# Human-Augment-Analytics/vectordb-retrieval

Measured on AMD Instinct MI355X. Metric: QPS @ recall@10 (SIFT1M-shaped, 10k-query batch, k=10), higher is better.
Workload: dtype i8 MFMA scan (i32 accumulate) + exact integer / f64 refine

## Files before the change

vectordb-retrieval_amd/csrc/scan_i8x16.hpp:

```cpp
#pragma once
#include "scan_i8.hpp"

namespace vdb {

__host__ __device__ inline int x16_row_in_span(int t, int rb, int m) { return (m >> 2) * 128 + t * 8 + rb * 4 + (m & 3); }

__device__ __forceinline__ int swap16(int v) { return __builtin_amdgcn_ds_swizzle(v, 0x401F); }

template <int KS2, int ST, int RING>
constexpr int scan_i8x16_lds_bytes() { return RING * (ST * 2 * KS2 * 64 * 16 + ST * 32 * 4); }

template <int KS2, int ST, int CB, int NWAVES = 8, int RING = 2, int AUX = 0>
__device__ __forceinline__ void scan_i8x16_body(const ScanI8Args &a, unsigned char *smem) {
    constexpr int NV = 2 * KS2;
    constexpr int NT = NWAVES * 64;
    constexpr int kStageVec = ST * NV * 64;
    constexpr int kBiasLoads = (ST * 32 + NT - 1) / NT;
    constexpr int TPS = kTilesPerSpan;
    constexpr int SPS = TPS / ST;
    constexpr int HC = CB / 2;
    constexpr int UNR = (ST * CB <= 16) ? ST : 1;
    static_assert(TPS % ST == 0 && ST >= 2 && CB % 2 == 0 && NWAVES <= 8, "bad geometry");
    static_assert(RING >= 2 && RING <= 8 && (RING == 2 || ST % 2 == 0), "bad ring");
    constexpr bool kDeep = RING > 2;
    static_assert(scan_i8x16_lds_bytes<KS2, ST, RING>() == RING * (kStageVec * 16 + ST * 32 * 4), "LDS size");
    const int mode = a.info->i8_mode;
    if (!mode) return;
    auto lds_a = [&](int buf) { return reinterpret_cast<int4v *>(smem + buf * (kStageVec * 16)); };
    auto lds_b = [&](int buf) { return reinterpret_cast<int *>(smem + RING * kStageVec * 16 + buf * (ST * 32 * 4)); };

    const int tid = threadIdx.x, lane = tid & 63;
    const int wave = __builtin_amdgcn_readfirstlane(tid >> 6);
    const int g = lane >> 4, h = g >> 1;
    const bool odd = (g & 1) != 0;
    const bool late = (NWAVES >= 2) && (wave >= NWAVES / 2);
    const int b = blockIdx.x;
    const int x = b & 7, jb = b >> 3;
    const int ci = jb / a.nqtiles, qt = jb - ci * a.nqtiles;
    const int chunk = x + 8 * ci;
    if (chunk >= a.nchunks) return;
    const int64_t q0 = (int64_t)qt * (NWAVES * 16 * CB) + wave * (16 * CB);
    const int64_t span0 = chunk_span0(chunk, a.spans_per_chunk, a.chunk_rem);
    int64_t span1 = chunk_span0(chunk + 1, a.spans_per_chunk, a.chunk_rem);
    if (span1 > a.nspans) span1 = a.nspans;
    const int64_t out_pitch = a.Qpad;
    const int64_t col0 = q0 + (odd ? 16 : 0) + (lane & 15);
    const int32_t *bias = a.bias8 + ((mode & 3) == 1 ? 0 : a.Npad);

    int4v bq[CB][KS2];
#pragma unroll
    for (int cb = 0; cb < CB; ++cb)
#pragma unroll
        for (int ks = 0; ks < KS2; ++ks) bq[cb][ks] = a.qpanels[((size_t)(q0 / 16 + cb) * KS2 + ks) * 64 + lane];
    const int nstages = (int)(span1 - span0) * SPS;
    const int INF = (int)kI8Inf;
    int m1[CB], m2[CB], M1[HC], M2[HC], Ms[HC];
#pragma unroll
    for (int cb = 0; cb < CB; ++cb) m1[cb] = m2[cb] = INF;
#pragma unroll
    for (int j = 0; j < HC; ++j) {
        M1[j] = M2[j] = INF;
        Ms[j] = 0;
    }

    constexpr int kPieces = kStageVec / 64;
    static_assert(kPieces % NWAVES == 0, "pieces must divide over the waves");
    constexpr int kBiasPieces = (ST / 2 + NWAVES - 1) / NWAVES;
    int stage_b[kBiasLoads];
    auto stage_issue = [&](int st, int buf) {
        const int64_t span = span0 + st / SPS;
        const int sq = st % SPS;
        const int4v *src = a.panels + ((size_t)(span * TPS + sq * ST) * NV) * 64;
        int4v *dst = lds_a(buf);
#pragma unroll
        for (int i = 0; i < kPieces / NWAVES; ++i) {
            const int p = wave + i * NWAVES;
            const int4v *gp = src + p * 64 + lane;
            __builtin_amdgcn_global_load_lds(
                reinterpret_cast<const __attribute__((address_space(1))) void *>(reinterpret_cast<uintptr_t>(gp)),
                reinterpret_cast<__attribute__((address_space(3))) void *>(
                    static_cast<uint32_t>(reinterpret_cast<uintptr_t>(dst + p * 64))),
                16, 0, AUX);
        }
        if (kDeep) {
#pragma unroll
            for (int i = 0; i < kBiasPieces; ++i) {
                const int j = (wave + i * NWAVES) % (ST / 2);
                const int t = 2 * j + (lane >> 5), gg = (lane >> 3) & 3, e = lane & 7;
                const int32_t *gp = bias + span * kSpanRows + gg * 128 + (sq * ST + t) * 8 + e;
                __builtin_amdgcn_global_load_lds(
                    reinterpret_cast<const __attribute__((address_space(1))) void *>(reinterpret_cast<uintptr_t>(gp)),
                    reinterpret_cast<__attribute__((address_space(3))) void *>(
                        static_cast<uint32_t>(reinterpret_cast<uintptr_t>(lds_b(buf) + j * 64))),
                    4, 0, 0);
            }
            return;
        }
#pragma unroll
        for (int i = 0; i < kBiasLoads; ++i) {
            const int e = tid + i * NT;
            if (e < ST * 32) {
                const int t = e >> 5, gg = (e >> 3) & 3, r = e & 7;
                stage_b[i] = bias[span * kSpanRows + gg * 128 + (sq * ST + t) * 8 + r];
            }
        }
    };
    auto stage_bias_store = [&](int buf) {
        if (kDeep) return;
#pragma unroll
        for (int i = 0; i < kBiasLoads; ++i)
            if (tid + i * NT < ST * 32) lds_b(buf)[tid + i * NT] = stage_b[i];
    };
    auto ring_issue = [&](int st) { stage_issue(st < nstages ? st : nstages - 1, st % RING); };
    auto ring_wait = [&]() {
        constexpr int kKeep = (RING - 2) * (kPieces / NWAVES + kBiasPieces);
        static_assert(kKeep < 64, "vmcnt is a 6-bit counter");
        asm volatile("s_waitcnt vmcnt(%0)" ::"n"(kKeep) : "memory");
        __builtin_amdgcn_s_barrier();
        asm volatile("" ::: "memory");
    };
    auto flush_bin = [&](int64_t span) {
        const size_t o = (size_t)(span * 2 + h) * out_pitch + col0;
#pragma unroll
        for (int j = 0; j < HC; ++j) {
            const int p1 = swap16(odd ? m1[2 * j] : m1[2 * j + 1]), p2 = swap16(odd ? m2[2 * j] : m2[2 * j + 1]);
            const int a1 = odd ? m1[2 * j + 1] : m1[2 * j], a2 = odd ? m2[2 * j + 1] : m2[2 * j];
            const int b1 = imin(a1, p1), b2 = imin(imax(a1, p1), imin(a2, p2));
            __builtin_nontemporal_store(__int_as_float(b1), a.bin_m1 + o + j * 32);
            __builtin_nontemporal_store(__int_as_float(b2), a.bin_m2 + o + j * 32);
            M2[j] = imin(imed3(M1[j], M2[j], b1), b2);
            if (b1 < M1[j]) Ms[j] = (int)span;
            M1[j] = imin(M1[j], b1);
        }
#pragma unroll
        for (int cb = 0; cb < CB; ++cb) m1[cb] = m2[cb] = INF;
    };

    if (kDeep) {
#pragma unroll
        for (int s = 0; s < RING - 1; ++s) ring_issue(s);
    } else {
        stage_issue(0, 0);
    }
    stage_bias_store(0);
    if (kDeep) ring_wait();
    else __syncthreads();

    if (a.nq_valid > 0 && q0 >= a.nq_valid) {
        for (int st = 0; st < nstages; ++st) {
            if (kDeep) {
                ring_issue(st + RING - 1);
                ring_wait();
                continue;
            }
            if (st + 1 < nstages) {
                stage_issue(st + 1, (st & 1) ^ 1);
                stage_bias_store((st & 1) ^ 1);
            }
            __syncthreads();
        }
        return;
    }

    int4v fr[NV], cin[2], acc[2][CB];
    auto read_phase = [&](const int4v *A_tile, const int4v *c_tile) {
#pragma unroll
        for (int v = 0; v < NV; ++v) fr[v] = A_tile[v * 64 + lane];
        cin[0] = c_tile[0];
        cin[1] = c_tile[1];
    };
    auto mfma_phase = [&]() {
#pragma unroll
        for (int ks = 0; ks < KS2; ++ks)
#pragma unroll
            for (int rb = 0; rb < 2; ++rb)
#pragma unroll
                for (int cb = 0; cb < CB; ++cb)
                    acc[rb][cb] = __builtin_amdgcn_mfma_i32_16x16x64_i8(fr[2 * ks + rb], bq[cb][ks], ks == 0 ? cin[rb] : acc[rb][cb], 0, 0, 0);
    };
    const unsigned id_hi = odd ? 16u : 0u;
    auto select_phase = [&](int t_bin) {
        const unsigned idv = (unsigned)__builtin_amdgcn_readfirstlane(t_bin) | id_hi;
#pragma unroll
        for (int cb = 0; cb < CB; ++cb) {
            const int t1 = imin(imin(acc[0][cb][0], acc[0][cb][1]), acc[0][cb][2]);
            const int t2 = imin(imin(acc[0][cb][3], acc[1][cb][0]), acc[1][cb][1]);
            const int q = imin(imin(imin(acc[1][cb][2], acc[1][cb][3]), t1), t2);
            const int v = (int)(((unsigned)q << 6) | idv);
            m2[cb] = imed3(m1[cb], m2[cb], v);
            m1[cb] = imin(m1[cb], v);
        }
    };
    if (a.prio == 1 && late) __builtin_amdgcn_s_setprio(1);
    else if (a.prio == 2 && !late) __builtin_amdgcn_s_setprio(1);
    if (!late) {
        for (int st = 0; st < nstages; ++st) {
            const int buf = kDeep ? st % RING : st & 1;
            if (kDeep) ring_issue(st + RING - 1);
            else if (st + 1 < nstages) stage_issue(st + 1, buf ^ 1);
            const int4v *A = lds_a(buf);
            const int4v *B4 = reinterpret_cast<const int4v *>(lds_b(buf)) + g * 2;
            const int ts0 = (st % SPS) * ST;
            read_phase(A, B4);
#pragma unroll UNR
            for (int t = 0; t < ST; ++t) {
                __builtin_amdgcn_sched_barrier(0);
                mfma_phase();
                __builtin_amdgcn_sched_barrier(0);
                if (t + 1 < ST) read_phase(A + (t + 1) * NV * 64, B4 + (t + 1) * 8);
                select_phase(ts0 + t);
            }
            __builtin_amdgcn_sched_barrier(0);
            if (ts0 + ST == TPS) flush_bin(span0 + st / SPS);
            if (!kDeep && st + 1 < nstages) stage_bias_store(buf ^ 1);
            if (kDeep) ring_wait();
            else __syncthreads();
        }
    } else {
#pragma unroll
        for (int rb = 0; rb < 2; ++rb)
#pragma unroll
            for (int cb = 0; cb < CB; ++cb)
#pragma unroll
                for (int r = 0; r < 4; ++r) acc[rb][cb][r] = (int)(kI8Inf >> 6);
        for (int st = 0; st < nstages; ++st) {
            const int buf = kDeep ? st % RING : st & 1;
            if (kDeep) ring_issue(st + RING - 1);
            else if (st + 1 < nstages) stage_issue(st + 1, buf ^ 1);
            const int4v *A = lds_a(buf);
            const int4v *B4 = reinterpret_cast<const int4v *>(lds_b(buf)) + g * 2;
            const int ts0 = (st % SPS) * ST;
#pragma unroll UNR
            for (int t = 0; t < ST; ++t) {
                __builtin_amdgcn_sched_barrier(0);
                read_phase(A + t * NV * 64, B4 + t * 8);
                select_phase((ts0 + t + TPS - 1) % TPS);
                if (t == 0 && st > 0 && ts0 == 0) flush_bin(span0 + st / SPS - 1);
                __builtin_amdgcn_sched_barrier(0);
                mfma_phase();
            }
            __builtin_amdgcn_sched_barrier(0);
            if (!kDeep && st + 1 < nstages) stage_bias_store(buf ^ 1);
            if (kDeep) ring_wait();
            else __syncthreads();
        }
        select_phase(TPS - 1);
        flush_bin(span1 - 1);
    }

    const size_t so = (size_t)(chunk * 2 + h) * a.Qpad + col0;
#pragma unroll
    for (int j = 0; j < HC; ++j) {
        a.sb_m1[so + j * 32] = __int_as_float(M1[j]);
        a.sb_m2[so + j * 32] = __int_as_float(M2[j]);
        a.sb_span[so + j * 32] = Ms[j];
    }
}

template <int KS2, int ST, int CB, int NWAVES = 8, int RING = 2, int AUX = 0>
__global__ __launch_bounds__(NWAVES * 64, (NWAVES >= 4 ? 2 : 1)) void scan_i8x16_kernel(ScanI8Args a) {
    __shared__ __attribute__((aligned(16))) unsigned char smem[scan_i8x16_lds_bytes<KS2, ST, RING>()];
    scan_i8x16_body<KS2, ST, CB, NWAVES, RING, AUX>(a, smem);
}

}
```

Measured before the change: 11.40 million.

## Software-pipeline i8x16 scan tiles with double-buffered accumulators and interleaved MFMA schedule

Adds a specialized batch loop for the 8-wave, 2-ring, non-unrolled configuration. Accumulators and fragments are double-buffered so the min-reduction and top-2 folds of the previous tile, plus the LDS reads for the next tile, interleave with the MFMAs of the current tile. sched_group_barrier patterns place VALU and DS ops into MFMA gaps. This aims to hide the select/fold VALU work and LDS latency behind matrix ops, at the cost of roughly doubling accumulator and fragment register use, which may reduce occupancy or cause spills.

```diff
diff --git a/vectordb-retrieval_amd/csrc/scan_i8x16.hpp b/vectordb-retrieval_amd/csrc/scan_i8x16.hpp
--- a/vectordb-retrieval_amd/csrc/scan_i8x16.hpp
+++ b/vectordb-retrieval_amd/csrc/scan_i8x16.hpp
@@ -9,6 +9,105 @@
 
 template <int KS2, int ST, int RING>
 constexpr int scan_i8x16_lds_bytes() { return RING * (ST * 2 * KS2 * 64 * 16 + ST * 32 * 4); }
+
+template <int N_MFMA, int N_VALU, int N_DS>
+__device__ __forceinline__ void x16_gap_pattern() {
+    constexpr int R = (N_VALU + N_DS + N_MFMA - 1) / N_MFMA;
+    static_assert(N_DS <= N_MFMA && R >= 2, "one LDS read per gap");
+#pragma unroll
+    for (int i = 0; i < N_MFMA; ++i) {
+        __builtin_amdgcn_sched_group_barrier(0x8, 1, 0);
+        if (i < N_DS) {
+            __builtin_amdgcn_sched_group_barrier(0x100, 1, 0);
+            __builtin_amdgcn_sched_group_barrier(0x2, R - 1, 0);
+        } else {
+            __builtin_amdgcn_sched_group_barrier(0x2, R, 0);
+        }
+    }
+}
+
+template <int KS2, int ST, int CB, class StageIssue, class BiasStore, class FlushBin>
+__device__ __forceinline__ void scan_i8x16_batch_loop(const unsigned char *smem, const int4v (&bq)[CB][KS2], int (&m1)[CB], int (&m2)[CB],
+                                                      int nstages, int64_t span0, int lane, StageIssue &&stage_issue,
+                                                      BiasStore &&stage_bias_store, FlushBin &&flush_bin) {
+    constexpr int NV = 2 * KS2, kStageVec = ST * NV * 64, TPS = kTilesPerSpan, SPS = TPS / ST;
+    constexpr int NM = 2 * KS2 * CB, NH = NM / 2;
+    static_assert(ST % 2 == 0 && TPS % ST == 0, "tile parity must be static in the unrolled stage");
+    const int g = lane >> 4;
+    const unsigned id_hi = (g & 1) ? 16u : 0u;
+    int4v acc[2][2][CB], fr[2][NV], cin[2][2];
+    int q[CB];
+#pragma unroll
+    for (int rb = 0; rb < 2; ++rb)
+#pragma unroll
+        for (int cb = 0; cb < CB; ++cb)
+#pragma unroll
+            for (int r = 0; r < 4; ++r) acc[1][rb][cb][r] = (int)(kI8Inf >> 6);
+    auto read_tile = [&](int p, const int4v *A, const int4v *B4, int t) {
+#pragma unroll
+        for (int v = 0; v < NV; ++v) fr[p][v] = A[(t * NV + v) * 64];
+        cin[p][0] = B4[t * 8];
+        cin[p][1] = B4[t * 8 + 1];
+    };
+    auto mfma_half = [&](int p, int half) {
+#pragma unroll
+        for (int m = half * NH; m < (half + 1) * NH; ++m) {
+            const int ks = m / (2 * CB), rb = (m / CB) % 2, cb = m % CB;
+            acc[p][rb][cb] = __builtin_amdgcn_mfma_i32_16x16x64_i8(fr[p][2 * ks + rb], bq[cb][ks], ks == 0 ? cin[p][rb] : acc[p][rb][cb], 0, 0, 0);
+        }
+    };
+    auto min_trees = [&](int o) {
+#pragma unroll
+        for (int cb = 0; cb < CB; ++cb) {
+            const int t1 = imin(imin(acc[o][0][cb][0], acc[o][0][cb][1]), acc[o][0][cb][2]);
+            const int t2 = imin(imin(acc[o][0][cb][3], acc[o][1][cb][0]), acc[o][1][cb][1]);
+            q[cb] = imin(imin(imin(acc[o][1][cb][2], acc[o][1][cb][3]), t1), t2);
+        }
+    };
+    auto folds = [&](int t_bin) {
+        const unsigned idv = (unsigned)__builtin_amdgcn_readfirstlane(t_bin) | id_hi;
+#pragma unroll
+        for (int cb = 0; cb < CB; ++cb) {
+            const int v = (int)(((unsigned)q[cb] << 6) | idv);
+            m2[cb] = imed3(m1[cb], m2[cb], v);
+            m1[cb] = imin(m1[cb], v);
+        }
+    };
+    for (int st = 0; st < nstages; ++st) {
+        const int buf = st & 1;
+        if (st + 1 < nstages) stage_issue(st + 1, buf ^ 1);
+        const int4v *A = reinterpret_cast<const int4v *>(smem + buf * (kStageVec * 16)) + lane;
+        const int4v *B4 = reinterpret_cast<const int4v *>(smem + 2 * kStageVec * 16 + buf * (ST * 32 * 4)) + g * 2;
+        const int ts0 = (st % SPS) * ST;
+        read_tile(0, A, B4, 0);
+#pragma unroll
+        for (int t = 0; t < ST; ++t) {
+            const int p = t & 1, o = p ^ 1;
+            __builtin_amdgcn_sched_barrier(0);
+            mfma_half(p, 0);
+            min_trees(o);
+            x16_gap_pattern<NH, 4 * CB, 0>();
+            __builtin_amdgcn_sched_barrier(0);
+#pragma unroll
+            for (int cb = 0; cb < CB; ++cb) asm volatile("" : "+v"(q[cb]));
+            __builtin_amdgcn_sched_barrier(0);
+            if (t + 1 < ST) read_tile(o, A, B4, t + 1);
+            mfma_half(p, 1);
+            folds((ts0 + t + TPS - 1) % TPS);
+            x16_gap_pattern<NH, 3 * CB + 1, NV + 2>();
+            __builtin_amdgcn_sched_barrier(0);
+#pragma unroll
+            for (int cb = 0; cb < CB; ++cb) asm volatile("" : "+v"(m1[cb]), "+v"(m2[cb]));
+            if (t == 0 && st > 0 && ts0 == 0) flush_bin(span0 + st / SPS - 1);
+        }
+        __builtin_amdgcn_sched_barrier(0);
+        if (st + 1 < nstages) stage_bias_store(buf ^ 1);
+        __syncthreads();
+    }
+    min_trees((ST - 1) & 1);
+    folds(TPS - 1);
+    flush_bin(span0 + nstages / SPS - 1);
+}
 
 template <int KS2, int ST, int CB, int NWAVES = 8, int RING = 2, int AUX = 0>
 __device__ __forceinline__ void scan_i8x16_body(const ScanI8Args &a, unsigned char *smem) {
@@ -162,6 +261,9 @@
         return;
     }
 
+    if constexpr (NWAVES == 8 && RING == 2 && UNR == 1) {
+        scan_i8x16_batch_loop<KS2, ST, CB>(smem, bq, m1, m2, nstages, span0, lane, stage_issue, stage_bias_store, flush_bin);
+    } else {
     int4v fr[NV], cin[2], acc[2][CB];
     auto read_phase = [&](const int4v *A_tile, const int4v *c_tile) {
 #pragma unroll
@@ -247,6 +349,7 @@
         select_phase(TPS - 1);
         flush_bin(span1 - 1);
     }
+    }
 
     const size_t so = (size_t)(chunk * 2 + h) * a.Qpad + col0;
 #pragma unroll
```

Result: faster. 11.75 million, median of 6 (+3.0%).
